# Illumina/Pisces

Measured on AMD Instinct MI355X. Metric: candidate loci/s at 500x depth, higher is better.
Workload: dtype int32 counts + f64 likelihoods; 1 GPU; BASELINE config 2: synthetic 100000 loci x 500x amplicon pileup, SNV-only, gVCF, per GPU per step; device-resident packed tuples; depth=500, ring_batches=6, tile_loci=56, parallelism=interval-shard x1

## Files before the change

### pisces_amd/csrc/kernels.hip.h

```cpp
#pragma once
#include <hip/hip_runtime.h>
#include <stdint.h>

#include "device_math.hip.h"
#include "genotype_core.h"

namespace pisces {

constexpr int kBlock = 256;
constexpr int kTile = 64;
constexpr int kFolded = 18;
constexpr int kUnroll = 8;
constexpr int kSlotsPerTile = 4 * kTile;
#ifndef PISCES_TOTAL_SHARDS
#define PISCES_TOTAL_SHARDS 64
#endif
constexpr int kTotalShards = PISCES_TOTAL_SHARDS;
constexpr int kTotalStride = 16;
constexpr int kRefMargin = 32;
constexpr int kRefWin = kTile + 2 * kRefMargin;
constexpr int kWaveRows = 32;
constexpr int kWaveRow = kTile;
constexpr int kWaveRegion = kWaveRows * kWaveRow;
constexpr int kQLutLds = 128;
// ... 135 lines not shown
    return point_counts_of(load_counts<H>(hist, l), allele, isRef, refType, gapped);
}

__device__ __forceinline__ bool variant_passes_frequency(const PointCounts& c, const DeviceParams& P)
{
    if (c.total < P.min_cov && !P.include_ref) return false;
    if (c.total != 0 && frequency_f(c.support, c.total) < P.min_freq) return false;
    return true;
}

struct GqPre { int32_t idx, val; };
template <bool kMemo = false>
__device__ inline bool finish_allele(const PointCounts& c, int pos, int a, bool isRef, int rt, int vq, const SbResult& sb,
                                     const uint8_t* __restrict__ ref, int64_t win_lo, int64_t win_hi, const DeviceParams& P,
                                     PiscesCalledAllele& r, const uint8_t* s_refwin, int s_refidx,
                                     const GqTail* pre_tail = nullptr, const GqPre* pre_gq = nullptr,
                                     const int32_t* window_level_ = nullptr )
{
    const float freq = frequency_f(c.support, c.total);
    const float allReads = (float)(c.total + c.nocalls);
    const float fractionNoCalls = (allReads == 0.0f) ? 0.0f : ((float)c.nocalls / allReads);
    uint32_t filters = 0;
    if (P.low_depth_filter >= 0 && c.total < P.low_depth_filter) filters |= 1u << PISCES_FILTER_LOW_DEPTH;
    if (P.vq_filter >= 0 && vq < P.vq_filter && c.total != 0) filters |= 1u << PISCES_FILTER_LOW_VARIANT_QSCORE;
    if (!isRef) {
        if (P.nocall_thr >= 0.0f && fractionNoCalls > P.nocall_thr) filters |= 1u << PISCES_FILTER_NO_CALL;
        if (!sb.acceptable || (P.filter_single_strand && !sb.var_both)) filters |= 1u << PISCES_FILTER_STRAND_BIAS;
        auto base_of = [](int code) { return (uint8_t)((0x54434741u >> (8 * code)) & 0xFFu); };
        if (rt < 4 && a < 4) {
            const bool hit = (s_refwin && P.rmxn_min_rep <= kRefMargin)
                                 ? rmxn_should_filter_snv_lds(s_refwin, kRefWin, s_refidx, base_of(rt), base_of(a), freq, P)
                                 : rmxn_should_filter_snv(ref, win_lo, win_hi, pos, base_of(rt), base_of(a), freq, P);
            if (hit) filters |= 1u << PISCES_FILTER_RMXN;
        }
        if (P.vf_filter >= 0.0f && freq < P.vf_filter) filters |= 1u << PISCES_FILTER_LOW_VARIANT_FREQUENCY;
    }
    const int gt = somatic_genotype(isRef, c.total, c.support, c.refsup, P);
    int gq;
    if (kMemo) {
        GqPre g;
        if (pre_gq) g = *pre_gq;
        else {
            g.idx = somatic_gq_index(gt, c.total, c.support, P);
            g.val = (g.idx >= 0 && P.gq_cap) ? (int32_t)P.gq_cap[g.idx] : 0;
        }
        if (!somatic_gq_try(gt, vq, c.total, c.support, P, g.idx, g.val, gq)) return false;
    } else {
        gq = pre_tail ? somatic_gq_finish(gt, vq, c.total, *pre_tail, P) : somatic_gq(gt, vq, c.total, c.support, P);
    }
    if (P.low_gq_filter >= 0 && (float)gq < (float)P.low_gq_filter) filters |= 1u << PISCES_FILTER_LOW_GENOTYPE_QUALITY;

    r.position = pos;
    r.total_coverage = c.total;
    r.allele_support = c.support;
    r.reference_support = c.refsup;
    r.num_no_calls = c.nocalls;
    r.coverage_by_dir[0] = c.cov[0]; r.coverage_by_dir[1] = c.cov[1]; r.coverage_by_dir[2] = c.cov[2];
    r.support_by_dir[0] = c.sup[0]; r.support_by_dir[1] = c.sup[1]; r.support_by_dir[2] = c.sup[2];
    r.variant_qscore = vq;
    r.strand_bias_score = sb.bias_score;
    r.genotype_qscore = (int16_t)gq;
    r.noise_level = c.support > 0 ? (window_level_ ? noise_level_field(*window_level_) : (int16_t)P.noise_level) : (int16_t)0;
    r.filter_bits = (uint16_t)filters;
    r.info = PISCES_INFO_PACK(gt, isRef ? PISCES_CAT_REFERENCE : PISCES_CAT_SNV, rt, isRef ? rt : a, sb.acceptable, sb.var_both,
                              sb.cov_both);
    return true;
}

template <bool kDiploidOk = false, bool kFinishAnyway = false>
__device__ inline bool process_point_allele(const PointCounts& c, int pos, int a, bool isRef, int rt,
                                             const uint8_t* __restrict__ ref, int64_t win_lo, int64_t win_hi,
                                             const DeviceParams& P, PiscesCalledAllele& r,
                                             const uint8_t* s_refwin = nullptr, int s_refidx = 0, const GqTail* pre_tail = nullptr,
                                             const int32_t* window_level_ = nullptr )
{
    bool callable = true;
    if (!isRef && !variant_passes_frequency(c, P)) {
        if (!kFinishAnyway) return false;
        callable = false;
    }
    int vq = 0;
    if (window_level_) {
        const double werr = window_err_of_level(*window_level_, P);
        if (c.support > 0 && c.total != 0 && werr >= 0.0) vq = poisson_qscore_e(c.support, c.total, werr, P);
    } else if (c.support > 0 && c.total != 0) {
        vq = poisson_qscore(c.support, c.total, P);
    }
    if (!isRef && vq < P.min_vq) {
        if (!kFinishAnyway) return false;
        callable = false;
    }
    SbResult sb = {0.0, 0, 0, 0};
    if (c.support > 0) sb = strand_bias<kDiploidOk>(c.cov, c.sup, P);
    finish_allele(c, pos, a, isRef, rt, vq, sb, ref, win_lo, win_hi, P, r, s_refwin, s_refidx, pre_tail, nullptr, window_level_);
    return callable;
}

struct VarScratch {
    int vq[kTile * 4];
    double ov_var[kTile * 4], fw_var[kTile * 4], fw_fp[kTile * 4], rv_var[kTile * 4], rv_fp[kTile * 4];
};

__device__ inline void call_roles(const int* hist, const uint32_t* gapped , const int32_t* s_lvl , const PiscesTile& tile,
                                  int tile_index, const uint8_t* __restrict__ ref, int32_t ref_start, int64_t ref_len,
                                  PiscesCalledAllele* __restrict__ records, PiscesTileResult* __restrict__ tile_result,
                                  const DeviceParams& P, uint8_t* s_mask ,
                                  const uint8_t* s_refwin , VarScratch* vs)
{
    const int wave = threadIdx.x >> 6;
    if (wave == 3) return;
    const int l = threadIdx.x & 63;
    const int pos = tile.start_position + l;
    const uint8_t refb = s_refwin[kRefMargin + l];
    const bool in_ref = l < tile.n_loci && refb != 0;
    const int rt = in_ref ? allele_type_of_base(refb) : PISCES_ALLELE_N;
    const int64_t win_lo = (int64_t)ref_start - 1, win_hi = win_lo + ref_len;
    const int g = gapped ? (int)gapped[l] : 0;
    PiscesCalledAllele* const slots = records + (int64_t)tile_index * kSlotsPerTile + l * 4;

    uint32_t pass_mask = 0;
    if (in_ref && rt < 4 && !P.refs_only && !locus_is_dirty(P, pos)) {
        for (int k = 0; k < 4; k++) {
            const int a = allele_of_rank(k);
            if (a == rt) continue;
            if (hist[(a * 3 + 0) * kTile + l] + hist[(a * 3 + 1) * kTile + l] + hist[(a * 3 + 2) * kTile + l] == 0) continue;
            const PointCounts c = point_counts(hist, l, a, false, rt, g);
            if (variant_passes_frequency(c, P)) pass_mask |= 1u << k;
        }
    }
    const bool tile_has_variants = __ballot(pass_mask != 0) != 0ull;
    if (!tile_has_variants && wave != 0) return;

    bool ref_emitted = false;
    int ref_rank = 0;
    if (wave == 0) {
        if (in_ref && P.include_ref) {
            int all = 0;
#pragma unroll
            for (int c = 0; c < kFolded; c++) all += hist[c * kTile + l];
            if (P.emit_zero_cov || all > 0) {
                const int a = (rt < 4) ? rt : PISCES_ALLELE_N;
                ref_rank = (rt < 4) ? rank_of_allele(rt) : 0;
                const PointCounts c = point_counts(hist, l, a, true, rt, g);
                PiscesCalledAllele rec;
                (void)process_point_allele<true>(c, pos, a, true, rt, ref, win_lo, win_hi, P, rec, s_refwin, kRefMargin + l, nullptr, s_lvl ? &s_lvl[l] : nullptr);
                copy_record(&slots[ref_rank], &rec);
                ref_emitted = true;
            }
        }
    } else {
        for (int k = 0; k < 4; k++) {
            if (!(pass_mask & (1u << k))) continue;
            const int a = allele_of_rank(k);
            const PointCounts c = point_counts(hist, l, a, false, rt, g);
            const int slot = l * 4 + k;
            if (wave == 1) {
                vs->vq[slot] = !(c.support > 0 && c.total != 0) ? 0 : !s_lvl ? poisson_qscore(c.support, c.total, P)
                               : s_lvl[l] != kNoLevel ? poisson_qscore_e(c.support, c.total, window_err_of_level(s_lvl[l], P), P) : 0;
            } else if (c.support > 0) {
                const SbStats ov = sb_stats_of<true>(0, c.cov, c.sup, P), fw = sb_stats_of<true>(1, c.cov, c.sup, P),
                              rv = sb_stats_of<true>(2, c.cov, c.sup, P);
                vs->ov_var[slot] = ov.var_gt_zero;
                vs->fw_var[slot] = fw.var_gt_zero; vs->fw_fp[slot] = fw.false_pos;
                vs->rv_var[slot] = rv.var_gt_zero; vs->rv_fp[slot] = rv.false_pos;
            }
        }
    }
    uint32_t vmask = 0;
    if (tile_has_variants) {
        __syncthreads();
        if (wave == 2) return;
        if (wave == 1) {
            uint32_t mask = 0;
            for (int k = 0; k < 4; k++) {
                if (!(pass_mask & (1u << k))) continue;
                const int a = allele_of_rank(k);
                const int slot = l * 4 + k;
                const int vq = vs->vq[slot];
                if (vq < P.min_vq) continue;
                const PointCounts c = point_counts(hist, l, a, false, rt, g);
                SbResult sb = {0.0, 0, 0, 0};
                if (c.support > 0) {
                    SbStats ov, fw, rv;
                    ov.var_gt_zero = vs->ov_var[slot];
                    fw.var_gt_zero = vs->fw_var[slot]; fw.false_pos = vs->fw_fp[slot];
                    rv.var_gt_zero = vs->rv_var[slot]; rv.false_pos = vs->rv_fp[slot];
                    const int s2 = c.sup[2] / 2, c2 = c.cov[2] / 2;
                    fw.coverage = c.cov[0] + c2; fw.support = c.sup[0] + s2;
                    rv.coverage = c.cov[1] + c2; rv.support = c.sup[1] + s2;
                    ov.false_pos = 0; ov.coverage = 0; ov.support = 0;
                    sb = sb_combine(ov, fw, rv, P);
                }
                PiscesCalledAllele r;
                finish_allele(c, pos, a, false, rt, vq, sb, ref, win_lo, win_hi, P, r, s_refwin, kRefMargin + l, nullptr, nullptr, s_lvl ? &s_lvl[l] : nullptr);
                copy_record(&slots[k], &r);
                mask |= 1u << k;
            }
            s_mask[l] = (uint8_t)mask;
        }
        __syncthreads();
        if (wave == 1) return;
        vmask = s_mask[l];
    }

    const uint32_t valid = vmask ? vmask : (ref_emitted ? (1u << ref_rank) : 0u);
    const int n_callable = __popc(vmask) + (ref_emitted ? 1 : 0);
    int n_surv = __popc(valid), n_call_total = n_callable;
#pragma unroll
    for (int d = 32; d >= 1; d >>= 1) {
        n_surv += __shfl_xor(n_surv, d, 64);
        n_call_total += __shfl_xor(n_call_total, d, 64);
    }
    const int n_loci_called = __popcll(__ballot(valid != 0));
    uint32_t word = valid << ((l & 7) * 4);
    word |= __shfl_xor(word, 1, 64);
    word |= __shfl_xor(word, 2, 64);
    word |= __shfl_xor(word, 4, 64);
    if ((l & 7) == 0) tile_result->valid[l >> 3] = word;
    if (l == 0) {
        tile_result->record_begin = tile_index * kSlotsPerTile;
        tile_result->n_records = n_surv;
        tile_result->n_candidate_loci = n_loci_called;
        tile_result->n_called = n_call_total;
        if (P.totals) {
            unsigned long long* tt = P.totals + (size_t)(tile_index % kTotalShards) * kTotalStride;
            atomicAdd(&tt[0], (unsigned long long)n_surv);
            atomicAdd(&tt[1], (unsigned long long)n_loci_called);
            atomicAdd(&tt[2], (unsigned long long)n_call_total);
            atomicAdd(&tt[3], 1ull);
        }
    }
}

__global__ __launch_bounds__(kBlock, 4) void call_tiles_kernel(
    const uint32_t* __restrict__ tuples, const PiscesTile* __restrict__ tiles, int32_t n_tiles,
    const uint8_t* __restrict__ ref, int32_t ref_start, int64_t ref_len, PiscesCalledAllele* __restrict__ records,
    PiscesTileResult* __restrict__ tile_results, DeviceParams P)
{
    __shared__ int hist[kFolded * kTile];
    __shared__ uint8_t s_mask[kTile];
    __shared__ uint8_t s_refwin[kRefWin];
    __shared__ VarScratch s_var;
    __shared__ double s_qlut[kQLutLds];

    const int t = blockIdx.x;
    if (t >= n_tiles) return;
    const PiscesTile tile = tiles[t];
#ifdef PISCES_TIMING
    const long long tc0 = wall_clock64();
#endif
    for (int i = threadIdx.x; i < kFolded * kTile; i += kBlock) hist[i] = 0;
    if (threadIdx.x < kRefWin) {
        const int64_t ri = (int64_t)tile.start_position - kRefMargin + threadIdx.x - ref_start;
        s_refwin[threadIdx.x] = (ri >= 0 && ri < ref_len) ? ref[ri] : (uint8_t)0;
    } else if (threadIdx.x >= 128 && threadIdx.x < 128 + kQLutLds) {
        const int q = threadIdx.x - 128;
        s_qlut[q] = (P.q_to_p_lut && q < P.q_to_p_n) ? P.q_to_p_lut[q] : q_to_p((double)q);
    }
    P.q_to_p_lut = s_qlut;
    P.q_to_p_n = kQLutLds;
    __syncthreads();

    const uint32_t n_loci = (uint32_t)tile.n_loci, min_bq = (uint32_t)P.min_bq;
    stream_tuples(tuples, tile.tuple_begin, tile.tuple_end,
                  [&](uint32_t v) { accumulate_folded(hist, v, n_loci, min_bq); });
    __syncthreads();
#ifdef PISCES_TIMING
    const long long tc1 = wall_clock64();
#endif
    call_roles(hist, nullptr, nullptr, tile, t, ref, ref_start, ref_len, records, &tile_results[t], P, s_mask, s_refwin, &s_var);
#ifdef PISCES_TIMING
    if (threadIdx.x == 0) {
        const long long tc2 = wall_clock64();
        tile_results[t].record_begin = (int)(tc0 & 0x3FFFFFFF);
        tile_results[t].n_records = (int)(tc1 & 0x3FFFFFFF);
        tile_results[t].n_candidate_loci = (int)(tc2 & 0x3FFFFFFF);
    }
#endif
}

#ifndef PISCES_WAVE_UNROLL
#define PISCES_WAVE_UNROLL 8
#endif
#ifndef PISCES_WAVE_OCC
#define PISCES_WAVE_OCC 3
#endif
#ifndef PISCES_WAVE2_OCC
#define PISCES_WAVE2_OCC 4
#endif
constexpr int kWaveUnroll = PISCES_WAVE_UNROLL;

template <int NW, typename Op, typename Pre>
__device__ __forceinline__ void stream_tuples_wave(const uint32_t* __restrict__ tuples, int64_t begin, int64_t end, int lane, int wid,
                                                   Op op, Pre pre)
{
    int64_t abegin = (begin + 3) & ~(int64_t)3;
    int64_t aend = end & ~(int64_t)3;
    if (abegin > aend) { abegin = end; aend = end; }
    const int tid = wid * 64 + lane;
    const u32x4* __restrict__ p4 = reinterpret_cast<const u32x4*>(tuples + abegin);
    const uint32_t n4 = (uint32_t)((aend - abegin) >> 2);
    constexpr uint32_t kBatch = 64u * kWaveUnroll;
    const uint32_t nb = (uint32_t)__builtin_amdgcn_readfirstlane((int)((n4 + kBatch - 1) / kBatch));
    u32x4 cur[kWaveUnroll], nxt[kWaveUnroll];
    auto load = [&](u32x4* v, uint32_t b) {
#pragma unroll
        for (int u = 0; u < kWaveUnroll; u++) {
            const uint32_t j = min(b * kBatch + (uint32_t)u * 64u + (uint32_t)lane, n4 - 1u);
            v[u] = __builtin_nontemporal_load(&p4[j]);
        }
    };
    auto consume = [&](const u32x4* v) {
#pragma unroll
        for (int u = 0; u < kWaveUnroll; u++) { op(v[u].x); op(v[u].y); op(v[u].z); op(v[u].w); }
    };
    const bool streams = (uint32_t)wid < nb;
    if (NW == 2) {
        if (streams) load(cur, (uint32_t)__builtin_amdgcn_readfirstlane(wid));
        __builtin_amdgcn_sched_barrier(0);
        pre();
    } else {
        pre();
        if (streams) load(cur, (uint32_t)__builtin_amdgcn_readfirstlane(wid));
    }
    for (int64_t i = begin + tid; i < abegin; i += 64 * NW) op(tuples[i]);
    if (streams) {
        uint32_t b = (uint32_t)__builtin_amdgcn_readfirstlane(wid);
        const uint32_t m = (nb - b + NW - 1) / NW;
        for (uint32_t p = (m - 1) / 2; p > 0; p--) {
            load(nxt, b + NW);
            __builtin_amdgcn_sched_barrier(0);
            consume(cur);
            __builtin_amdgcn_sched_barrier(0);
            load(cur, b + 2 * NW);
            __builtin_amdgcn_sched_barrier(0);
            consume(nxt);
            __builtin_amdgcn_sched_barrier(0);
            b += 2 * NW;
        }
        if (((m - 1) & 1u) != 0) {
            load(nxt, b + NW);
            __builtin_amdgcn_sched_barrier(0);
            consume(cur);
            __builtin_amdgcn_sched_barrier(0);
#pragma unroll
            for (int u = 0; u < kWaveUnroll; u++) cur[u] = nxt[u];
            b += NW;
        }
        if (b == nb - 1 && (n4 % kBatch)) {
#pragma unroll
            for (int u = 0; u < kWaveUnroll; u++)
                if (b * kBatch + (uint32_t)u * 64u + (uint32_t)lane >= n4) cur[u] = (u32x4){~0u, ~0u, ~0u, ~0u};
        }
        consume(cur);
    }
    for (int64_t i = aend + tid; i < end; i += 64 * NW) op(tuples[i]);
}

__device__ __forceinline__ void wave_lds_sync()
{
    __builtin_amdgcn_fence(__ATOMIC_SEQ_CST, "workgroup");
    __builtin_amdgcn_wave_barrier();
}

template <typename H = HistWave>
__device__ __forceinline__ uint32_t slow_alleles(const int* hist, const uint8_t* s_refwin, uint32_t slow, int l, int pos, int rt, int ref_rank,
                                                 const uint8_t* __restrict__ ref, int64_t win_lo, int64_t win_hi, PiscesCalledAllele* slots,
                                                 const DeviceParams& P)
{
    uint32_t called = 0;
    const int ref_a = (rt < 4) ? rt : PISCES_ALLELE_N;
#pragma unroll 1
    for (int k = 0; k < 5; k++) {
        if (!((slow >> k) & 1u)) continue;
        const bool isRef = k == 4;
        const int a = isRef ? ref_a : allele_of_rank(k);
        const LocusCounts lc = load_counts_wave<H>(hist, l);
        const PointCounts c = point_counts_of(lc, a, isRef, rt, 0);
        int vq = 0;
        if (c.support > 0 && c.total != 0) vq = poisson_qscore_out_of_line(c.support, c.total, P.err_q, P.max_vq, P.ln10);
        if (!isRef && vq < P.min_vq) continue;
        SbResult sb = {0.0, 0, 0, 0};
        if (c.support > 0) sb = strand_bias_out_of_line(c.cov, c.sup, P);
        PiscesCalledAllele r;
        (void)finish_allele<false>(c, pos, a, isRef, rt, vq, sb, ref, win_lo, win_hi, P, r, s_refwin, kRefMargin + l);
        copy_record(&slots[isRef ? ref_rank : k], &r);
        if (!isRef) called |= 1u << k;
    }
    return called;
}

template <int NW, typename H = HistWave>
__device__ __forceinline__ void call_phase_wave(const int* hist, const uint8_t* s_refwin, uint8_t* s_vmask, const PiscesTile& tile, const int t,
                                                const int l, const int wid, const uint8_t* __restrict__ ref, const int32_t ref_start,
                                                const int64_t ref_len, PiscesCalledAllele* __restrict__ records,
                                                PiscesTileResult* __restrict__ tile_results, const DeviceParams& P
#ifdef PISCES_TIMING
                                                , const long long tc0, const long long tc1
#endif
                                                )
{
    const int pos = tile.start_position + l;
    const uint8_t refb = s_refwin[kRefMargin + l];
    const bool in_ref = l < tile.n_loci && refb != 0;
    const int rt = in_ref ? allele_type_of_base(refb) : PISCES_ALLELE_N;
    const int64_t win_lo = (int64_t)ref_start - 1, win_hi = win_lo + ref_len;
    auto slot_of = [&](int k) { return records + ((int64_t)t * kSlotsPerTile + l * 4 + k); };
    const bool dirty = locus_is_dirty(P, pos);
    const LocusCounts lc = load_counts_wave<H>(hist, l);
    const bool ref_wave = wid == 0, var_wave = wid == NW - 1;
    if (P.folded_out && ref_wave && l < tile.n_loci) {
        const unsigned rel = (unsigned)(pos - P.folded_first);
        if (rel < (unsigned)P.folded_n) {
            int32_t* const dst = P.folded_out + (size_t)rel * PISCES_FOLDED_PER_LOCUS;
#pragma unroll
            for (int a = 0; a < 6; a++)
#pragma unroll
                for (int d = 0; d < 3; d++) dst[a * 3 + d] = lc.h[a][d];
        }
    }

    const bool tabs = tables_complete(P);
    auto fast_allele = [&](const PointCounts& c, int a, bool isRef, PiscesCalledAllele& rec) -> bool {
        int vq = 0;
        double sb_score = 0.0;
        int sb_ok = 0, sb_var = 0, sb_cov = 0;
        if (!tabs) return false;
        const AlleleTables tb = request_allele_tables(isRef, c.support, c.total, c.refsup, c.cov, c.sup, P);
        if (c.support > 0 && c.total != 0 && !poisson_qscore_try(c.support, c.total, P, tb, vq)) return false;
        if (!isRef && vq < P.min_vq) return true;
        if (c.support > 0 && !strand_bias_try(c.cov, c.sup, P, tb, sb_score, sb_ok, sb_var, sb_cov)) return false;
        const GqPre g = {tb.gq_idx, tb.gq_cap};
        const SbResult sb = {sb_score, sb_ok, sb_var, sb_cov};
        if (!finish_allele<true>(c, pos, a, isRef, rt, vq, sb, ref, win_lo, win_hi, P, rec, s_refwin, kRefMargin + l, nullptr, &g)) return false;
        return true;
    };
    bool ref_emitted = false;
    int ref_rank = 0;
    uint32_t slow = 0;
    uint32_t vmask = 0;
    const int ref_a = (rt < 4) ? rt : PISCES_ALLELE_N;
    if (ref_wave) {
        const PointCounts c = point_counts_of(lc, ref_a, true, rt, 0);
        if (in_ref && P.include_ref && !P.variants_only && (P.emit_zero_cov || c.total + c.nocalls > 0)) {
            ref_rank = (rt < 4) ? rank_of_allele(rt) : 0;
            ref_emitted = true;
            PiscesCalledAllele rec;
            if (fast_allele(c, ref_a, true, rec)) copy_record(slot_of(ref_rank), &rec);
            else slow |= 16u;
        }
    }
#ifdef PISCES_TIMING
    const long long tcA = wall_clock64();
#endif
    if (var_wave && in_ref && rt < 4 && !P.refs_only && !dirty) {
#pragma unroll 1
        for (int k = 0; k < 4; k++) {
            const int a = allele_of_rank(k);
            if (a == rt) continue;
            const PointCounts c = point_counts_of(lc, a, false, rt, 0);
            if (c.support == 0) continue;
            if (!variant_passes_frequency(c, P)) continue;
            PiscesCalledAllele r;
            r.position = 0;
            if (!fast_allele(c, a, false, r)) { slow |= 1u << k; continue; }
            if (r.position == 0) continue;
            copy_record(slot_of(k), &r);
            vmask |= 1u << k;
        }
    }
    if (__builtin_expect(__ballot(slow != 0) != 0ull, 0))
        vmask |= slow_alleles<H>(hist, s_refwin, slow, l, pos, rt, ref_rank, ref, win_lo, win_hi, records + ((int64_t)t * kSlotsPerTile + l * 4), P);
    if (NW == 2) {
        if (var_wave) s_vmask[l] = (uint8_t)vmask;
        __syncthreads();
        if (!ref_wave) return;
        vmask = s_vmask[l];
    }
#ifdef PISCES_TIMING
    const long long tcB = wall_clock64();
#endif

    const uint32_t valid = vmask ? vmask : (ref_emitted ? (1u << ref_rank) : 0u);
    int n_surv = 0, n_var = 0;
#pragma unroll
    for (int k = 0; k < 4; k++) {
        n_surv += __popcll(__ballot((valid >> k) & 1u));
        n_var += __popcll(__ballot((vmask >> k) & 1u));
    }
    const int n_call_total = n_var + __popcll(__ballot(ref_emitted));
    const int n_loci_called = __popcll(__ballot(valid != 0));
    uint32_t word = valid << ((l & 7) * 4);
    word |= __shfl_xor(word, 1, 64);
    word |= __shfl_xor(word, 2, 64);
    word |= __shfl_xor(word, 4, 64);
    PiscesTileResult* const tile_result = &tile_results[t];
    if ((l & 7) == 0) tile_result->valid[l >> 3] = word;
    if (l == 0) {
        tile_result->record_begin = t * kSlotsPerTile;
        tile_result->n_records = n_surv;
        tile_result->n_candidate_loci = n_loci_called;
        tile_result->n_called = n_call_total;
        if (P.totals) {
            unsigned long long* tt = P.totals + (size_t)(t % kTotalShards) * kTotalStride;
            atomicAdd(&tt[0], (unsigned long long)n_surv);
            atomicAdd(&tt[1], (unsigned long long)n_loci_called);
            atomicAdd(&tt[2], (unsigned long long)n_call_total);
            atomicAdd(&tt[3], 1ull);
        }
#ifdef PISCES_TIMING
        const long long tc2 = wall_clock64();
        tile_result->record_begin = (int)(tc0 & 0x3FFFFFFF);
        tile_result->n_records = (int)(tc1 & 0x3FFFFFFF);
        tile_result->n_candidate_loci = (int)(tc2 & 0x3FFFFFFF);
        tile_result->n_called = (int)__builtin_amdgcn_s_getreg(63492);
        tile_result->valid[0] = __builtin_amdgcn_s_getreg(63508);
        tile_result->valid[1] = 0;
        tile_result->valid[2] = (uint32_t)(tcA - tc1);
        tile_result->valid[3] = (uint32_t)(tcB - tcA);
        tile_result->valid[4] = 0;
        tile_result->valid[5] = (uint32_t)(tc2 - tcB);
#endif
    }
}

template <int NW>
__global__ __launch_bounds__(64 * NW, NW == 1 ? PISCES_WAVE_OCC : PISCES_WAVE2_OCC) void call_tiles_wave_kernel(
    const uint32_t* __restrict__ tuples, const PiscesTile* __restrict__ tiles, int32_t n_tiles,
    const uint8_t* __restrict__ ref, int32_t ref_start, int64_t ref_len, PiscesCalledAllele* __restrict__ records,
    PiscesTileResult* __restrict__ tile_results, DeviceParams P, const DeviceParams* __restrict__ Pd )
{
    __shared__ __attribute__((aligned(16))) int hist[2 * kWaveRegion];
    __shared__ uint8_t s_refwin[kRefWin];
    __shared__ uint8_t s_vmask[kTile];

    const int t = blockIdx.x;
    if (t >= n_tiles) return;
    const int l = threadIdx.x & 63, wid = threadIdx.x >> 6;
    const PiscesTile tile = tiles[t];
#ifdef PISCES_TIMING
    const long long tc0 = wall_clock64();
#endif
    auto setup = [&]() {
        int4* h4 = reinterpret_cast<int4*>(hist);
        for (int i = threadIdx.x; i < 2 * kWaveRegion / 4; i += 64 * NW) h4[i] = make_int4(0, 0, 0, 0);
        for (int i = threadIdx.x; i < kRefWin; i += 64 * NW) {
            const int64_t ri = (int64_t)tile.start_position - kRefMargin + i - ref_start;
            s_refwin[i] = (ri >= 0 && ri < ref_len) ? ref[ri] : (uint8_t)0;
        }
        __syncthreads();
    };

    {
        if (NW == 2) __builtin_amdgcn_s_setprio(3);
        const uint32_t min_bq_shifted = (uint32_t)min(max(P.min_bq, 0), 255) << 24;
        stream_tuples_wave<NW>(tuples, tile.tuple_begin, tile.tuple_end, l, wid, [&](uint32_t v) { accumulate_wave(hist, v, min_bq_shifted); }, setup);
    }
    __syncthreads();
    if (NW == 2) __builtin_amdgcn_s_setprio(0);
#ifdef PISCES_TIMING
    const long long tc1 = wall_clock64();
#endif

    call_phase_wave<NW>(hist, s_refwin, s_vmask, tile, t, l, wid, ref, ref_start, ref_len, records, tile_results, P
#ifdef PISCES_TIMING
                        , tc0, tc1
#endif
                        );
}

__global__ __launch_bounds__(256) void build_vq_tab_kernel(int16_t* __restrict__ tab, int32_t n_k, int32_t n_cov, DeviceParams P)
{
    const int64_t i = (int64_t)blockIdx.x * blockDim.x + threadIdx.x;
    if (i >= (int64_t)n_k * n_cov) return;
    tab[i] = (int16_t)poisson_qscore((int32_t)(i / n_cov), (int32_t)(i % n_cov), P);
}
__global__ __launch_bounds__(256) void build_sb_tab_kernel(double* __restrict__ tab, double* __restrict__ tab0, int32_t n_k, int32_t n_cov, DeviceParams P)
{
    const int64_t i = (int64_t)blockIdx.x * blockDim.x + threadIdx.x;
    if (i >= (int64_t)n_k * n_cov) return;
    const int k = (int)(i / n_cov), cov = (int)(i % n_cov);
    tab[i] = k >= 1 ? fmax(0.0, poisson_cdf_sb((double)k - 1, (double)cov * P.err_sb)) : 0.0;
    if (k == 0) tab0[cov] = pow(1 - P.err_sb, (double)cov);
}
__global__ __launch_bounds__(256) void build_gq_cap_kernel(int16_t* __restrict__ tab, const double* __restrict__ gq_tail, int32_t n_a, int32_t n_cov, DeviceParams P)
{
    const int64_t i = (int64_t)blockIdx.x * blockDim.x + threadIdx.x;
    if (i >= (int64_t)n_a * n_cov) return;
    if (i < n_cov) { tab[i] = 0; return; }
    double rawQ = p_to_q(q_to_p_int(P.max_vq, P) + gq_tail[i]);
    double qScore = fmin((double)P.max_gq, rawQ);
    qScore = fmax(qScore, (double)P.min_gq);
    tab[i] = (int16_t)rint(qScore);
}

__global__ __launch_bounds__(64) void totals_collect_kernel(unsigned long long* __restrict__ shards, unsigned long long* __restrict__ out_host, int reset)
{
    const int l = threadIdx.x;
    if (l < 4) {
        unsigned long long v = 0;
        for (int sh = 0; sh < kTotalShards; sh++) v += shards[sh * kTotalStride + l];
        out_host[l] = v;
    }
    if (reset)
        for (int i = l; i < kTotalShards * kTotalStride; i += 64) shards[i] = 0ull;
    __threadfence_system();
}

__global__ __launch_bounds__(256) void read_probe_kernel(const u32x4* __restrict__ p, int64_t n4, uint32_t* __restrict__ sink)
{
    uint32_t acc = 0;
    const int64_t stride = (int64_t)gridDim.x * blockDim.x * 8;
    for (int64_t i = (int64_t)blockIdx.x * blockDim.x * 8 + threadIdx.x; i < n4; i += stride) {
        u32x4 v[8];
#pragma unroll
        for (int u = 0; u < 8; u++) {
            const int64_t j = i + (int64_t)u * blockDim.x;
            v[u] = j < n4 ? __builtin_nontemporal_load(&p[j]) : (u32x4){0u, 0u, 0u, 0u};
        }
#pragma unroll
        for (int u = 0; u < 8; u++) acc ^= v[u].x ^ v[u].y ^ v[u].z ^ v[u].w;
    }
    if (acc == 0x9E3779B9u) *sink = acc;
}

__global__ __launch_bounds__(256) void read_probe_dword_kernel(const uint32_t* __restrict__ p, int64_t n, uint32_t* __restrict__ sink)
{
    uint32_t acc = 0;
    const int64_t stride = (int64_t)gridDim.x * blockDim.x * 8;
    for (int64_t i = (int64_t)blockIdx.x * blockDim.x * 8 + threadIdx.x; i < n; i += stride) {
        uint32_t v[8];
#pragma unroll
        for (int u = 0; u < 8; u++) {
            const int64_t j = i + (int64_t)u * blockDim.x;
            v[u] = j < n ? p[j] : 0u;
        }
#pragma unroll
        for (int u = 0; u < 8; u++) acc ^= v[u];
    }
    if (acc == 0x9E3779B9u) *sink = acc;
}

__global__ void build_gq_tail_kernel(double* __restrict__ table, int32_t n_a, int32_t n_cov, float target_lod)
{
    const int64_t i = (int64_t)blockIdx.x * blockDim.x + threadIdx.x;
    if (i >= (int64_t)n_a * n_cov) return;
    const int a = (int)(i / n_cov), cov = (int)(i % n_cov);
    const float expectedF = target_lod * (float)cov;
    table[i] = a >= 1 ? incomplete_gamma_function((double)a, (double)expectedF) : -1.0;
}

template <typename T, typename R>
__host__ __device__ inline R anchor_adjusted(const T* __restrict__ row, int minAnchor, int maxAnchor, bool fromEnd)
{
    const int wellAnchoredIndex = PISCES_ANCHOR_SIZE, numAnchorIndexes = PISCES_NUM_ANCHORS;
    const int trueMinAnchor = wellAnchoredIndex < minAnchor ? wellAnchoredIndex : minAnchor;
    int initialMaxAnchor = wellAnchoredIndex;
// ... 710 lines not shown
```

Measured before the change: 2.561 billion candidate loci/s.

## Triple-buffer wave tuple streaming and shift partial batch to the front

The wave-level tuple streamer moves from a two-buffer ping-pong to three rotating register buffers, so two batches of loads are in flight while one is consumed. The batch grid is also offset backwards so that the partial batch comes first. Only the first load needs clamping and masking, and the steady-state loads drop the per-element min clamp. This costs more vector registers per wave, which could lower occupancy.

```diff
diff --git a/pisces_amd/csrc/kernels.hip.h b/pisces_amd/csrc/kernels.hip.h
--- a/pisces_amd/csrc/kernels.hip.h
+++ b/pisces_amd/csrc/kernels.hip.h
@@ -461,57 +461,80 @@
     const uint32_t n4 = (uint32_t)((aend - abegin) >> 2);
     constexpr uint32_t kBatch = 64u * kWaveUnroll;
     const uint32_t nb = (uint32_t)__builtin_amdgcn_readfirstlane((int)((n4 + kBatch - 1) / kBatch));
-    u32x4 cur[kWaveUnroll], nxt[kWaveUnroll];
+    const int rem = (int)(n4 % kBatch);
+    const int off = rem ? rem - (int)kBatch : 0;
+    u32x4 xa[kWaveUnroll], xb[kWaveUnroll], xc[kWaveUnroll];
     auto load = [&](u32x4* v, uint32_t b) {
-#pragma unroll
-        for (int u = 0; u < kWaveUnroll; u++) {
-            const uint32_t j = min(b * kBatch + (uint32_t)u * 64u + (uint32_t)lane, n4 - 1u);
-            v[u] = __builtin_nontemporal_load(&p4[j]);
-        }
+        const u32x4* __restrict__ q = p4 + (off + (int)(b * kBatch) + lane);
+#pragma unroll
+        for (int u = 0; u < kWaveUnroll; u++) v[u] = __builtin_nontemporal_load(q + u * 64);
+    };
+    auto load_first = [&](u32x4* v, uint32_t b) {
+#pragma unroll
+        for (int u = 0; u < kWaveUnroll; u++) v[u] = __builtin_nontemporal_load(&p4[max(off + (int)(b * kBatch) + u * 64 + lane, 0)]);
     };
     auto consume = [&](const u32x4* v) {
 #pragma unroll
         for (int u = 0; u < kWaveUnroll; u++) { op(v[u].x); op(v[u].y); op(v[u].z); op(v[u].w); }
+    };
+    auto step = [&](u32x4* x, uint32_t b) {
+        consume(x);
+        __builtin_amdgcn_sched_barrier(0);
+        load(x, b);
+        __builtin_amdgcn_sched_barrier(0);
+    };
+    auto mask_batch0 = [&](u32x4* v) {
+        if (wid == 0 && rem) {
+#pragma unroll
+            for (int u = 0; u < kWaveUnroll; u++)
+                if (off + u * 64 + lane < 0) v[u] = (u32x4){~0u, ~0u, ~0u, ~0u};
+        }
     };
     const bool streams = (uint32_t)wid < nb;
     if (NW == 2) {
-        if (streams) load(cur, (uint32_t)__builtin_amdgcn_readfirstlane(wid));
+        if (streams) load_first(xa, (uint32_t)__builtin_amdgcn_readfirstlane(wid));
         __builtin_amdgcn_sched_barrier(0);
         pre();
     } else {
         pre();
-        if (streams) load(cur, (uint32_t)__builtin_amdgcn_readfirstlane(wid));
+        if (streams) load_first(xa, (uint32_t)__builtin_amdgcn_readfirstlane(wid));
     }
     for (int64_t i = begin + tid; i < abegin; i += 64 * NW) op(tuples[i]);
     if (streams) {
         uint32_t b = (uint32_t)__builtin_amdgcn_readfirstlane(wid);
         const uint32_t m = (nb - b + NW - 1) / NW;
-        for (uint32_t p = (m - 1) / 2; p > 0; p--) {
-            load(nxt, b + NW);
+        if (m >= 3) {
+            load(xb, b + NW);
+            load(xc, b + 2 * NW);
             __builtin_amdgcn_sched_barrier(0);
-            consume(cur);
+            mask_batch0(xa);
+            for (uint32_t p = (m - 3) / 3; p > 0; p--) {
+                step(xa, b + 3 * NW);
+                step(xb, b + 4 * NW);
+                step(xc, b + 5 * NW);
+                b += 3 * NW;
+            }
+            const uint32_t r3 = (m - 3) % 3;
+            if (r3 == 0) {
+                consume(xa); consume(xb); consume(xc);
+                asm volatile("; stream tail 0");
+            } else if (r3 == 1) {
+                step(xa, b + 3 * NW);
+                consume(xb); consume(xc); consume(xa);
+                asm volatile("; stream tail 1");
+            } else {
+                step(xa, b + 3 * NW);
+                step(xb, b + 4 * NW);
+                consume(xc); consume(xa); consume(xb);
+                asm volatile("; stream tail 2");
+            }
+        } else {
+            if (m == 2) load(xb, b + NW);
             __builtin_amdgcn_sched_barrier(0);
-            load(cur, b + 2 * NW);
-            __builtin_amdgcn_sched_barrier(0);
-            consume(nxt);
-            __builtin_amdgcn_sched_barrier(0);
-            b += 2 * NW;
-        }
-        if (((m - 1) & 1u) != 0) {
-            load(nxt, b + NW);
-            __builtin_amdgcn_sched_barrier(0);
-            consume(cur);
-            __builtin_amdgcn_sched_barrier(0);
-#pragma unroll
-            for (int u = 0; u < kWaveUnroll; u++) cur[u] = nxt[u];
-            b += NW;
-        }
-        if (b == nb - 1 && (n4 % kBatch)) {
-#pragma unroll
-            for (int u = 0; u < kWaveUnroll; u++)
-                if (b * kBatch + (uint32_t)u * 64u + (uint32_t)lane >= n4) cur[u] = (u32x4){~0u, ~0u, ~0u, ~0u};
-        }
-        consume(cur);
+            mask_batch0(xa);
+            consume(xa);
+            if (m == 2) consume(xb);
+        }
     }
     for (int64_t i = aend + tid; i < end; i += 64 * NW) op(tuples[i]);
 }
```

Measured after the change: 2.585 billion candidate loci/s, median of 6. About the same (+0.9%).
